# Harounnn/Clustering-Driven-Replication-Strategy

Hardware: AMD Instinct MI355X
Metric: Lloyd point-iters/sec (whole node) + achieved HBM GB/s, 100M files d=16 k=64 (higher is better)
Workload: dtype f64

## Files before the change

### clustering-driven-replication-strategy_amd/csrc/screen32b.hip

```cpp
#include "screen32_common.h"
#include "screen32_fix.h"

namespace cdr {

template <int Q, int MT>
__global__ __launch_bounds__(256, 4) void screen32b(S32BArgs B) {
  const S32PArgs& a = B.p;
  constexpr int QH = FixDims<Q>::QH;
  if (a.gate && a.gate[0] == 0) return;
  constexpr bool H1 = QH == 1;
  constexpr int kTile = H1 ? 512 : 1024;
  constexpr int kHalf = kTile / 2;
  constexpr int kPB = H1 ? 8 : 16;
  constexpr int NWH = kPB / 4;
  constexpr int kRow = 2 * kPB;
  typedef unsigned u4v __attribute__((ext_vector_type(4)));
  __shared__ __attribute__((aligned(16))) float c32s[64 * kPrStr + 128];
  float* const eb = c32s + 64 * kPrStr;
  float* const hc = eb + 64;
  constexpr size_t kQBytes = 4 * 2 * 2 * kTile + 4 * 128 * sizeof(int2);
  __shared__ __attribute__((aligned(16))) unsigned char qlds[kQBytes > kFixLdsBytes ? kQBytes : kFixLdsBytes];
  typedef unsigned char QRow[2][2 * kTile];
  QRow* qd = reinterpret_cast<QRow*>(qlds);
  int2 (*qm)[128] = reinterpret_cast<int2 (*)[128]>(qlds + 4 * 2 * 2 * kTile);
// ... 133 lines not shown
    const int label = (int)(bA & 63u);
    const float vb = __uint_as_float(bA & ~63u);
    const float vs = __uint_as_float(sA_ & ~63u);
    float thr = fmaf(vb, thr_rel, thr0);
    unsigned ua = __float_as_uint(hA), ub = __float_as_uint(hB);
    swap32(ua, ub);
    const float hsum = __uint_as_float(ua) + __uint_as_float(ub);
    const float hh = fmaf(hsum, 1.0f + 0x1p-18f, 0x1p-20f);
    const float hl = hsum * (1.0f - 0x1p-18f);
    const float dn = fmaf(0x1p-11f * (1.0f + 0x1p-9f), __builtin_amdgcn_sqrtf(hh), 0x1p-23f);
    {
      const float K = thr0 + hh - Dlo;
      const float Gs = fmaxf(vs + K, 0x1p-100f), Gb = fmaxf(fmaf(vb, thr_rel, K), 0x1p-100f);
      thr += 2.0f * (1.0f + 0x1p-19f) * dn * (__builtin_amdgcn_sqrtf(Gs) + __builtin_amdgcn_sqrtf(Gb));
    }
    const bool valid = lane < nvalid;
    const bool cert = vs > thr;
    const int pt = meta.x, ob = meta.y;
    const bool moved = valid && cert && label != ob;
    if (moved) {
      a.labels[pt] = label;
      a.lab8[pt] = (uint8_t)label;
    }
    const float gb = fmaf(vb, thr_rel, thr0 + hh - Dlo);
    const float gs = vs - ((thr0 + Dhi) - hl);
    const float u0 = fmaf(__builtin_amdgcn_sqrtf(fmaxf(gb, 0.0f)), 1.0f + 0x1p-19f, dn);
    const float l0 = fmaf(__builtin_amdgcn_sqrtf(fmaxf(gs, 0.0f)), 1.0f - 0x1p-19f, -dn);
    const float wl = __shfl(wdn_l, label);
    if (valid) B.zb[pt] = cert ? zb_pack(l0, u0, wl, (unsigned)label) : (kZbStale | (unsigned)ob);
    const bool unc = valid && !cert;
    const unsigned long long mv = __ballot(moved);
    const unsigned long long need = __ballot(unc);
    const int rm = __builtin_amdgcn_mbcnt_hi((unsigned)(mv >> 32),
                                             __builtin_amdgcn_mbcnt_lo((unsigned)mv, 0u));
    const int rn = __builtin_amdgcn_mbcnt_hi((unsigned)(need >> 32),
                                             __builtin_amdgcn_mbcnt_lo((unsigned)need, 0u));
    if (moved) mv_region[mv_used + rm] = int2{pt, ob | (label << 16)};
    if (unc) fb_region[fb_used + rn] = int2{pt, ob};
    mv_used += __popcll(mv);
    fb_used += __popcll(need);
  };
  int qh = 0, qn = 0;
  int qtot = 0, ttot = 0;
  auto process = [&](const Row& b, bool valid, int pt, int ao) __attribute__((always_inline)) {
    const float qa = dist2(b, ao);
    const float uba = fmaf(__builtin_amdgcn_sqrtf(qa), 1.0f + 0x1p-18f, eb[ao]);
    const float l0 = fmaf(hc[ao], 1.0f - 0x1p-22f, -uba);
    const bool keep = l0 > uba * (1.0f + 0x1p-20f);
    if (valid && keep) B.zb[pt] = zb_pack(l0, uba, __shfl(wdn_l, ao), (unsigned)ao);
#ifdef CDR_EXPERIMENTS
    const bool q = valid && !keep && !(B.dbg & 8);
#else
    const bool q = valid && !keep;
#endif
    const unsigned long long m = __ballot(q);
    if (m) {
      if (q) {
        const int r = __builtin_amdgcn_mbcnt_hi((unsigned)(m >> 32),
                                                __builtin_amdgcn_mbcnt_lo((unsigned)m, 0u));
        const int slot = (qh + r) & 127;
        const int e = slot & 63;
        unsigned char* dst = qd[wv][slot >> 6] + (e >> 5) * kTile + (e & 31) * kPB;
        if constexpr (H1) {
          *reinterpret_cast<uint2*>(dst) = uint2{b.w[0], b.w[1]};
          *reinterpret_cast<uint2*>(dst + kHalf) = uint2{b.w[2], b.w[3]};
        } else {
          *reinterpret_cast<uint4*>(dst) = uint4{b.w[0], b.w[1], b.w[2], b.w[3]};
          *reinterpret_cast<uint4*>(dst + kHalf) = uint4{b.w[4], b.w[5], b.w[6], b.w[7]};
        }
        qm[wv][slot] = int2{pt, ao};
      }
      const int c = __popcll(m);
      qh = (qh + c) & 127;
      qn += c;
      qtot += c;
      if (qn >= 64) {
        drain(((qh - qn) & 127) >> 6, 64);
        qn -= 64;
      }
    }
  };
  unsigned* const fl = flist[wv];
  struct GB {
    Row r;
    int pt, ao;
    bool valid;
  };
  auto gload = [&](GB& g, int b, int cnt) __attribute__((always_inline)) {
    const int e = 64 * b + lane;
    g.valid = e < cnt;
    const unsigned ent = fl[g.valid ? e : 64 * b];
    const int64_t ci = wave + (int64_t)(ent >> 14) * nwaves;
    const int64_t pt = ci * kBChunk + ((ent >> 6) & 255);
    g.pt = (int)pt;
    g.ao = (int)(ent & 63);
    const u4v* src = reinterpret_cast<const u4v*>(B.XH + pt * kRow);
    const u4v q0 = __builtin_nontemporal_load(src);
    g.r.w[0] = q0.x; g.r.w[1] = q0.y; g.r.w[2] = q0.z; g.r.w[3] = q0.w;
    if constexpr (!H1) {
      const u4v q1 = __builtin_nontemporal_load(src + 1);
      g.r.w[4] = q1.x; g.r.w[5] = q1.y; g.r.w[6] = q1.z; g.r.w[7] = q1.w;
    }
  };
  auto phase2 = [&](int& cnt, bool last) __attribute__((always_inline)) {
    const int nb = last ? (cnt + 63) >> 6 : cnt >> 6;
    if (nb == 0) return;
    ttot += last ? cnt : nb * 64;
#ifdef CDR_EXPERIMENTS
    if (B.dbg & 4) {
      cnt = 0;
      return;
    }
#endif
    GB g[3];
    gload(g[0], 0, cnt);
    gload(g[1], nb > 1 ? 1 : 0, cnt);
    for (int b = 0; b < nb; b += 3) {
#pragma unroll
      for (int i = 0; i < 3; ++i) {
        const int nx = b + i + 2;
        gload(g[(i + 2) % 3], nx < nb ? nx : nb - 1, cnt);
        if (b + i < nb) process(g[i].r, g[i].valid, g[i].pt, g[i].ao);
      }
    }
    const int done = nb * 64;
    const int rem = last ? 0 : cnt - done;
    if (rem > 0) {
      const unsigned v = lane < rem ? fl[done + lane] : 0u;
      __builtin_amdgcn_wave_barrier();
      if (lane < rem) fl[lane] = v;
    }
    cnt = rem;
  };

  int cnt = 0;
  int64_t it = 0;
  for (int64_t C0 = wave; C0 < nchunks; C0 += (int64_t)kBPD * nwaves) {
#pragma unroll
    for (int i = 0; i < kBPD; ++i, ++it) {
      const int64_t Ci = C0 + (int64_t)i * nwaves;
      if (Ci >= nchunks) break;
      zload(zc[(i + kBPD - 1) % kBPD], Ci + (int64_t)(kBPD - 1) * nwaves);
      const u4v z = zc[i];
#pragma unroll
      for (int u = 0; u < 4; ++u) {
        const unsigned w = z[u];
        const unsigned lab = w & 63u;
#ifdef CDR_EXPERIMENTS
        const bool fail = (!(__uint_as_float(w & ~63u) > __shfl(wup_l, (int)lab)) || (B.dbg & 1)) &&
                          !(B.dbg & 16);
#else
        const bool fail = !(__uint_as_float(w & ~63u) > __shfl(wup_l, (int)lab)) || (B.dbg & 1);
#endif
        const unsigned long long m = __ballot(fail);
        if (m) {
          if (fail) {
            const int r = __builtin_amdgcn_mbcnt_hi((unsigned)(m >> 32),
                                                    __builtin_amdgcn_mbcnt_lo((unsigned)m, 0u));
            fl[cnt + r] = (unsigned)it << 14 | (unsigned)(4 * lane + u) << 6 | lab;
          }
          cnt += __popcll(m);
        }
      }
      if (cnt > kBList - kBChunk) phase2(cnt, false);
    }
  }
  phase2(cnt, true);
  if (qn > 0) drain(((qh - qn) & 127) >> 6, qn);
  if (lane == 0) {
    a.fb_count[wave] = fb_used;
    a.mv_count[wave] = mv_used;
    if (a.q_acc) a.q_acc[wave] += qtot;
    if (B.t_acc) B.t_acc[wave] += ttot;
  }
#ifdef CDR_EXPERIMENTS
  if (B.dbg & 2) return;
#endif
  if (!a.fuse) return;
  __syncthreads();
  const FixLds L(qlds);
  if (lane == 0) {
    L.s_mv[wv + 1] = mv_used;
    L.s_fb[wv + 1] = fb_used;
  }
  fixup_regions<Q, MT>(a.fx, blockIdx.x * 4, 4, blockIdx.x % kRunSlices, L, FixPlan{sA, sC});
}

template <int KPD>
__global__ __launch_bounds__(256) void screen32bz(S32BArgs B) {
  const S32PArgs& a = B.p;
  if (a.gate && a.gate[0] == 0) return;
  typedef unsigned u4v __attribute__((ext_vector_type(4)));
  constexpr int kZList = KPD * kBChunk + 64;
  __shared__ unsigned flist[4][kZList];
  const int t = threadIdx.x;
  const int lane = t & 63;
  const int wv = t >> 6;
  const int wave = __builtin_amdgcn_readfirstlane(blockIdx.x * 4 + wv);
  const int64_t nchunks = B.nchunks;
  int64_t wbase, wend;
  int wstride;
  bs_range(B, wv, wbase, wstride, wend);
  auto zload = [&](u4v& z, int64_t ci) __attribute__((always_inline)) {
    const int64_t cc = ci < nchunks ? ci : nchunks - 1;
    z = __builtin_nontemporal_load(reinterpret_cast<const u4v*>(B.zb + cc * kBChunk) + lane);
  };
  u4v zc[KPD];
#pragma unroll
  for (int i = 0; i < KPD - 1; ++i) zload(zc[i], wbase + (int64_t)i * wstride);
  const float wup_l = B.wup[lane];
  unsigned* const fl = flist[wv];
  uint32_t* const out = B.zl + (size_t)wave * B.zcap;
  int cnt = 0, total = 0;
  int it = 0;
  for (int64_t C0 = wbase; C0 < wend; C0 += (int64_t)KPD * wstride) {
#pragma unroll
    for (int i = 0; i < KPD; ++i, ++it) {
      const int64_t Ci = C0 + (int64_t)i * wstride;
      if (Ci >= wend) break;
      zload(zc[(i + KPD - 1) % KPD], Ci + (int64_t)(KPD - 1) * wstride);
      const u4v z = zc[i];
#pragma unroll
      for (int u = 0; u < 4; ++u) {
        const unsigned w = z[u];
        const unsigned lab = w & 63u;
        const bool fail = !(__uint_as_float(w & ~63u) > __shfl(wup_l, (int)lab)) || (B.dbg & 1);
        const unsigned long long m = __ballot(fail);
        if (m) {
          if (fail) {
            const int r = __builtin_amdgcn_mbcnt_hi((unsigned)(m >> 32),
                                                    __builtin_amdgcn_mbcnt_lo((unsigned)m, 0u));
            fl[cnt + r] = (unsigned)it << 14 | (unsigned)(4 * lane + u) << 6 | lab;
          }
          cnt += __popcll(m);
        }
      }
    }
    if (cnt >= 64) {
      const int full = cnt & ~63;
      __builtin_amdgcn_wave_barrier();
      for (int o = 0; o < full; o += 64) out[total + o + lane] = fl[o + lane];
      const int rem = cnt - full;
      const unsigned v = lane < rem ? fl[full + lane] : 0u;
      __builtin_amdgcn_wave_barrier();
      if (lane < rem) fl[lane] = v;
      total += full;
      cnt = rem;
    }
  }
  __builtin_amdgcn_wave_barrier();
  if (lane < cnt) out[total + lane] = fl[lane];
  if (lane == 0) B.zn[wave] = total + cnt;
}

__global__ void zb_reset_kernel(const uint8_t* __restrict__ lab8, uint32_t* __restrict__ zb,
                                int64_t n, int64_t n_pad, const long long* __restrict__ gate) {
  if (gate && gate[0] == 0) return;
  for (int64_t i = (int64_t)blockIdx.x * blockDim.x + threadIdx.x; i < n_pad;
       i += (int64_t)gridDim.x * blockDim.x)
    zb[i] = i < n ? (kZbStale | lab8[i]) : 0x7F000000u;
}

__global__ void zh_reset_kernel(const uint8_t* __restrict__ lab8, uint16_t* __restrict__ zh,
                                int64_t n, int64_t n_pad, const long long* __restrict__ gate) {
  if (gate && gate[0] == 0) return;
  for (int64_t i = (int64_t)blockIdx.x * blockDim.x + threadIdx.x; i < n_pad;
       i += (int64_t)gridDim.x * blockDim.x)
    zh[i] = i < n ? (uint16_t)lab8[i] : (uint16_t)kZ16Pad;
}

__device__ __forceinline__ unsigned zb16_rebase(unsigned w, float dg, int e0o, int e0n) {
  const unsigned c = w >> 6;
  if (c == 0u || c == 1023u) return w;
  const float t = zb16_dec((int)c, e0o) - dg;
  int cn = t > 0.0f ? zb16_code(t * (1.0f - 0x1p-22f), e0n) : -1;
  cn = cn < 0 ? 0 : (cn > 1022 ? 1022 : cn);
  return (unsigned)cn << 6 | (w & 63u);
}

__global__ __launch_bounds__(256) void zh_rebase_kernel(uint16_t* __restrict__ zh, int64_t n_pad,
                                                        const unsigned char* __restrict__ bt,
                                                        const long long* __restrict__ gate) {
  if (gate && gate[0] == 0) return;
  const int* hd = reinterpret_cast<const int*>(bt + kBndHdr);
  if (hd[3] == 0) return;
  __shared__ float dgs[64];
  if (threadIdx.x < 64) dgs[threadIdx.x] = reinterpret_cast<const float*>(bt + kBndDG)[threadIdx.x];
  __syncthreads();
  const int e0o = hd[1], e0n = hd[2];
  typedef unsigned u4v __attribute__((ext_vector_type(4)));
  u4v* z4 = reinterpret_cast<u4v*>(zh);
  for (int64_t i = (int64_t)blockIdx.x * blockDim.x + threadIdx.x; i < n_pad / 8;
       i += (int64_t)gridDim.x * blockDim.x) {
    u4v z = __builtin_nontemporal_load(z4 + i);
#pragma unroll
    for (int q = 0; q < 4; ++q) {
      const unsigned lo = z[q] & 0xFFFFu, hi = z[q] >> 16;
      z[q] = zb16_rebase(lo, dgs[lo & 63u], e0o, e0n) | zb16_rebase(hi, dgs[hi & 63u], e0o, e0n) << 16;
    }
    __builtin_nontemporal_store(z, z4 + i);
  }
}

__global__ __launch_bounds__(256) void zh_watch_kernel(uint16_t* __restrict__ zh, int64_t n_pad,
                                                       unsigned char* __restrict__ bt,
                                                       const long long* __restrict__ gate,
                                                       uint32_t* __restrict__ wl,
                                                       int32_t* __restrict__ wn, int wcap,
                                                       int wrange) {
  if (gate && gate[0] == 0) return;
  const int* hd = reinterpret_cast<const int*>(bt + kBndHdr);
  int* wh = reinterpret_cast<int*>(bt + kBndWatch);
  const bool reb = hd[3] != 0;
  if (!reb && (wh[kWFin] == kWatchList || wh[kWHold])) return;
  __shared__ float dgs[64];
  __shared__ unsigned hs[64];
  const int t = threadIdx.x, lane = t & 63;
  if (t < 64) {
    dgs[t] = reinterpret_cast<const float*>(bt + kBndDG)[t];
    hs[t] = reinterpret_cast<const unsigned*>(bt + kBndH)[t];
  }
  __syncthreads();
  if (blockIdx.x == 0) {
    if (t < 64) reinterpret_cast<unsigned*>(bt + kBndHL)[t] = hs[t];
    if (t == 0) {
      wh[kWMode] = kWatchList;
      wh[kWValid] = 1;
      wh[kWEpochs] += 1;
      if (reb) wh[kWCarried] += 1;
    }
  }
  const int e0o = hd[1], e0n = hd[2];
  typedef unsigned u4v __attribute__((ext_vector_type(4)));
  const int wave = blockIdx.x * 4 + (t >> 6);
  const int64_t p0 = (int64_t)wave * wrange;
  const int64_t p1 = p0 + wrange < n_pad ? p0 + wrange : n_pad;
  uint32_t* const out = wl + (size_t)wave * wcap;
  int cnt = 0;
  constexpr int kU = 4;
  for (int64_t c0 = p0; c0 < p1; c0 += kU * kZ16Chunk) {
    u4v z[kU];
#pragma unroll
    for (int i = 0; i < kU; ++i) {
      const int64_t ci = c0 + i * kZ16Chunk < p1 ? c0 + i * kZ16Chunk : c0;
      z[i] = __builtin_nontemporal_load(reinterpret_cast<const u4v*>(zh + ci) + lane);
    }
#pragma unroll
    for (int i = 0; i < kU; ++i) {
      const int64_t ci = c0 + i * kZ16Chunk;
      if (ci >= p1) break;
      if (reb) {
#pragma unroll
        for (int q = 0; q < 4; ++q) {
          const unsigned lo = z[i][q] & 0xFFFFu, hi = z[i][q] >> 16;
          z[i][q] = zb16_rebase(lo, dgs[lo & 63u], e0o, e0n) |
                    zb16_rebase(hi, dgs[hi & 63u], e0o, e0n) << 16;
        }
        __builtin_nontemporal_store(z[i], reinterpret_cast<u4v*>(zh + ci) + lane);
      }
      const unsigned off = (unsigned)(ci - p0) + 8u * (unsigned)lane;
#pragma unroll
      for (int u = 0; u < 8; ++u) {
        const unsigned w = (z[i][u >> 1] >> (16 * (u & 1))) & 0xFFFFu;
        const bool listed = (w >> 6) <= hs[w & 63u];
        const unsigned long long m = __ballot(listed);
        if (m) {
          const int r = cnt + __builtin_amdgcn_mbcnt_hi((unsigned)(m >> 32),
                                                        __builtin_amdgcn_mbcnt_lo((unsigned)m, 0u));
          if (listed && r < wcap) out[r] = (off + (unsigned)u) << 16 | w;
          cnt += __popcll(m);
        }
      }
    }
  }
  if (lane == 0) {
    wn[wave] = cnt < wcap ? cnt : wcap;
    if (cnt > wcap) wh[kWOvf] = 1;
  }
}

void zh_rebase(Ctx& c, const long long* gate) {
  if (!c.zb_valid || c.zb_fmt != 16 || !c.bnd_ok) return;
  if (c.watch_on)
    hipLaunchKernelGGL(zh_watch_kernel, dim3(c.watch_waves / 4), dim3(256), 0, c.stream,
                       c.zb.as<uint16_t>(), c.n_pad, static_cast<unsigned char*>(c.bnd.p), gate,
                       c.wl.as<uint32_t>(), c.wn.as<int32_t>(), c.watch_cap, c.watch_range);
  else
    hipLaunchKernelGGL(zh_rebase_kernel, dim3(2048), dim3(256), 0, c.stream, c.zb.as<uint16_t>(),
                       c.n_pad, reinterpret_cast<const unsigned char*>(c.bnd.p), gate);
  HIP_CHECK(hipGetLastError());
}

void bound_words_reset(bool z16, hipStream_t s, const uint8_t* lab8, void* zb, int64_t n,
                       int64_t n_pad, const long long* gate) {
  if (z16)
    hipLaunchKernelGGL(zh_reset_kernel, dim3(2048), dim3(256), 0, s, lab8,
                       static_cast<uint16_t*>(zb), n, n_pad, gate);
  else
    hipLaunchKernelGGL(zb_reset_kernel, dim3(2048), dim3(256), 0, s, lab8,
                       static_cast<uint32_t*>(zb), n, n_pad, gate);
}

int screen32b_blocks_per_cu(int Q, int MT) {
  static int cache[4][2] = {};
  int& nb = cache[Q - 1][MT - 1];
  if (!nb)
    dispatch_q_mt<4>(Q, MT, [&](auto q, auto m) {
      nb = occupancy_blocks(screen32b<decltype(q)::value, decltype(m)::value>, 0);
    });
  return nb;
}

void screen32b_launch(int Q, int MT, dim3 grid, hipStream_t s, const S32BArgs& p) {
  dispatch_q_mt<4>(Q, MT, [&](auto q, auto m) {
    hipLaunchKernelGGL((screen32b<decltype(q)::value, decltype(m)::value>), grid, dim3(256), 0, s, p);
  });
}

void screen32bz_launch(dim3 grid, hipStream_t s, const S32BArgs& p) {
  static const int pd = exp_env("CDR_S32BZ_PD") ? std::atoi(exp_env("CDR_S32BZ_PD")) : 8;
  if (pd == 4) hipLaunchKernelGGL(screen32bz<4>, grid, dim3(256), 0, s, p);
  else if (pd == 12) hipLaunchKernelGGL(screen32bz<12>, grid, dim3(256), 0, s, p);
  else hipLaunchKernelGGL(screen32bz<8>, grid, dim3(256), 0, s, p);
}

}
```

### clustering-driven-replication-strategy_amd/csrc/screen32bs_body.h

```cpp
  static_assert(!(SPLIT && WATCH) && (!WATCH || CDR_S32BS_LAZY), "the WATCH form: 2-byte words, lazy phase 2");
  const S32PArgs& a = B.p;
  const FixArgs& F = a.fx;
#ifdef CDR_EXPERIMENTS
  unsigned long long tp[8] = {__builtin_amdgcn_s_memrealtime(), 0, 0, 0, 0, 0, 0, 0};
#define CDR_TP(i) tp[i] = __builtin_amdgcn_s_memrealtime()
#else
#define CDR_TP(i)
#endif
  constexpr int QH = FixDims<Q>::QH;
  constexpr int DM = FixDims<Q>::DM;
#ifndef CDR_S32BS_DEFER
#define CDR_S32BS_DEFER 1
#endif
  constexpr bool DEFER = !SPLIT && CDR_S32BS_DEFER;
  if constexpr (!MERGED) {
  if (!SPLIT && B.dyn && blockIdx.x == 0 && threadIdx.x < 32)
    B.dyn[((B.dyn_par ^ 1) * 32 + threadIdx.x) * 32] = 0u;
  if (a.gate && a.gate[0] == 0) return;
  if constexpr (!SPLIT) {
    if (B.watch) {
      const bool list = B.watch[kWMode] == kWatchList && B.watch[kWOvf] == 0;
      if (list != WATCH) return;
      if (blockIdx.x == 0 && threadIdx.x == 0) {
        B.watch[WATCH ? kWListN : kWFullN] += 1;
        B.watch[kWLast] = WATCH ? kWatchList : kWatchFull;
      }
    }
  }
  }
  typedef unsigned u4v __attribute__((ext_vector_type(4)));
  typedef float f2 __attribute__((ext_vector_type(2)));
  float* const eb = c32s + 64 * kPrStr;
  float* const hc = eb + 64;
  const int t = threadIdx.x;
  const int lane = t & 63;
  const int wv = t >> 6;
  const int h = lane >> 5, p = lane & 31;
  const int wave = __builtin_amdgcn_readfirstlane(blockIdx.x * 4 + wv);
  const int64_t nchunks = B.nchunks;
  const int k = a.k, d = a.d, d1 = d + 1;
  if constexpr (MERGED) __builtin_assume(d > 4 * (Q - 1));
  uint32_t* const wlw = WATCH ? B.wl + (size_t)wave * B.wcap : nullptr;
  const int pbase = WATCH ? wave * B.wrange : 0;

  constexpr int CH = SPLIT ? kBChunk : kZ16Chunk;
  constexpr int SH = SPLIT ? 14 : 15;
  auto zload = [&](u4v& z, int64_t ci) __attribute__((always_inline)) {
    const int64_t cc = ci < nchunks ? ci : nchunks - 1;
    z = __builtin_nontemporal_load(reinterpret_cast<const u4v*>(B.zh + cc * kZ16Chunk) + lane);
  };
  int64_t wbase, wend;
  int wstride;
  int64_t rR0 = 0;
  int rsl = 0;
  bs_range(B, wv, wbase, wstride, wend, &rR0, &rsl);
  const bool dyn = !SPLIT && !WATCH && B.dyn != nullptr && B.slot_wg > 0;
  int swend = (int)wend, P0 = (int)wend, P1 = (int)wend;
  if (dyn) {
    const int spw = (int)((wend - rR0) * B.dyn_pct / 100 / wstride);
    swend = (int)rR0 + spw * wstride;
    const int xcd = blockIdx.x & 7;
    P0 = swend + (int)((wend - swend) * xcd / 8);
    P1 = swend + (int)((wend - swend) * (xcd + 1) / 8);
  }
  const int ebase = dyn ? (int)rR0 : (int)wbase;
  const int estride = dyn ? 1 : wstride;
  u4v zc[kBPD];

  constexpr int kPr4 = (64 * kPrStr + 128) / 4;
  static_assert(kPr4 <= 512 && MT * 2 * 64 <= 256, "prologue: two float4 per thread");
  const f4* prune4 = reinterpret_cast<const f4*>(a.prune);
  const f4 pv0 = prune4[t];
  const f4 pv1 = t + 256 < kPr4 ? prune4[t + 256] : f4{0.f, 0.f, 0.f, 0.f};
  h8 av = {};
  if (t < MT * 2 * 64) av = a.frag[t];
  float cv = 0.0f;
  const int cm = t >> 5, ci4 = (t >> 3) & 3, chh = (t >> 2) & 1, cc = t & 3;
  if (t < MT * 32) cv = a.cinit[(cm * 16 + ci4 * 4 + cc) * 64 + chh * 32];
  float wup_l = 0.0f, wnew_l;
  int e0n = 0;
  if constexpr (SPLIT) {
    wup_l = B.wup[lane];
    wnew_l = B.wdn[lane];
  } else {
    wnew_l = reinterpret_cast<const float*>(B.bt + kBndWdg)[lane];
    e0n = reinterpret_cast<const int*>(B.bt + kBndHdr)[2];
  }
  auto zput = [&](int pt, int sl, bool ok, float l0, float u0, float w, unsigned lab) __attribute__((always_inline)) {
    if constexpr (SPLIT) {
      B.zb[pt] = ok ? zb_pack(l0, u0, w, lab) : (kZbStale | lab);
    } else {
      const unsigned short w16 = ok ? zb16_pack(l0, u0, w, e0n, lab) : (unsigned short)lab;
      B.zh[pt] = w16;
      if constexpr (WATCH) wlw[sl] = (unsigned)(pt - pbase) << 16 | w16;
    }
  };
  const float msv = lane < d ? F.ms[lane] : 0.0f;
  const float thr0 = a.thr_dev ? a.thr_dev[0] : a.thr0, thr_rel = a.thr_rel;
  const float Dv = a.thr_dev ? a.thr_dev[1] : a.Dv;
  const float Dlo = Dv * (1.0f - 0x1p-19f), Dhi = Dv * (1.0f + 0x1p-19f);
  const float sig = F.sig;
  int wtotal = 0;
  unsigned tlv = 0;
  if constexpr (WATCH) {
    wtotal = B.wn[wave];
    if (t < 64) tlv = (B.dbg & 1) ? 1022u : reinterpret_cast<const unsigned*>(B.bt + kBndT)[t];
    const int lastl = (B.wcap >> 8) - 1;
    const u4v* const wl4 = reinterpret_cast<const u4v*>(wlw);
#pragma unroll
    for (int i = 0; i < kBPD; ++i) {
      __builtin_amdgcn_sched_barrier(0);
      zc[i] = wl4[(size_t)(i < lastl ? i : lastl) * 64 + lane];
    }
    __builtin_amdgcn_sched_barrier(0);
    if (t < 64) tls[t] = tlv;
  }
  reinterpret_cast<f4*>(c32s)[t] = pv0;
  if (t + 256 < kPr4) reinterpret_cast<f4*>(c32s)[t + 256] = pv1;
  if (t < MT * 2 * 64) sA[t] = av;
  if (t < MT * 32) sC[t] = cv;
  for (int e = t; e < 64 * 17; e += 256) mtab[e] = 0ull;
  if (t < 16) msl[t] = msv;
  if constexpr (!SPLIT && !WATCH) {
    if (t < 64) tls[t] = (B.dbg & 1) ? 1022u : reinterpret_cast<const unsigned*>(B.bt + kBndT)[t];
  }
  if constexpr (WATCH) wtotal = __builtin_amdgcn_readfirstlane(wtotal);
  __syncthreads();
  CDR_TP(1);

  int fb_used = 0, fb_cert = 0, mv_used = 0, qtot = 0, ttot = 0;
  const f4* XA4 = reinterpret_cast<const f4*>(F.XA);

  auto screen_m = [&](int m, const u4v (&v)[QH]) __attribute__((always_inline)) -> f16v {
    asm volatile("" ::: "memory");
    const h8 A0 = sA[(m * 2 + 0) * 64 + lane];
    const h8 A1 = sA[(m * 2 + 1) * 64 + lane];
    f16v acc;
#pragma unroll
    for (int i4 = 0; i4 < 4; ++i4) {
      const f4 c4v = *reinterpret_cast<const f4*>(sC + ((m * 4 + i4) * 2 + h) * 4);
#pragma unroll
      for (int i = 0; i < 4; ++i) acc[4 * i4 + i] = c4v[i];
    }
    const h8 BH = __builtin_bit_cast(h8, v[0]);
    acc = __builtin_amdgcn_mfma_f32_32x32x16_f16(A0, BH, acc, 0, 0, 0);
    if constexpr (QH == 2) {
      const h8 BL = __builtin_bit_cast(h8, v[QH - 1]);
      acc = __builtin_amdgcn_mfma_f32_32x32x16_f16(A0, BL, acc, 0, 0, 0);
    }
    return __builtin_amdgcn_mfma_f32_32x32x16_f16(A1, BH, acc, 0, 0, 0);
  };
  auto tile = [&](const u4v (&v)[QH], unsigned& bk, unsigned& sk) __attribute__((always_inline)) {
    unsigned b = 0xFFFFFFFFu, s = 0xFFFFFFFFu;
#pragma nounroll
    for (int m = 0; m < MT; ++m) {
      const f16v acc = screen_m(m, v);
      const unsigned rb = 32u * (unsigned)m;
      auto key = [&](int i) {
        return (__float_as_uint(acc[i]) & ~63u) | (rb + (unsigned)(8 * (i >> 2) + (i & 3)));
      };
#pragma unroll
      for (int q = 0; q < 16; q += 2) {
        const unsigned x = key(q), y = key(q + 1);
        unsigned tq;
        asm("v_med3_u32 %0, %1, %2, %3" : "=v"(tq) : "v"(b), "v"(x), "v"(y));
        asm("v_min3_u32 %0, %1, %2, %3" : "=v"(b) : "v"(b), "v"(x), "v"(y));
        s = min(s, tq);
      }
    }
    bk = b | ((unsigned)h << 2);
    sk = s | ((unsigned)h << 2);
  };
  auto cmask = [&](const u4v (&v)[QH], float tau) __attribute__((always_inline)) -> unsigned {
    unsigned r = 0;
#pragma nounroll
    for (int m = 0; m < MT; ++m) {
      const f16v acc = screen_m(m, v);
#pragma unroll
      for (int i = 0; i < 16; ++i) {
        const float kv = __uint_as_float(__float_as_uint(acc[i]) & ~63u);
        if (!(kv > tau)) r |= 1u << (16 * m + i);
      }
    }
    return r;
  };
  auto q32 = [&](const float (&xh)[DM], int j) __attribute__((always_inline)) -> float {
    const f4* c4 = reinterpret_cast<const f4*>(c32s + j * kPrStr);
    f2 acc = {0.0f, 0.0f};
#pragma unroll
    for (int q = 0; q < Q; ++q) {
      const f4 cq = c4[q];
#pragma unroll
      for (int u = 0; u < 2; ++u) {
        const f2 df = {xh[4 * q + 2 * u] - cq[2 * u], xh[4 * q + 2 * u + 1] - cq[2 * u + 1]};
        acc = __builtin_elementwise_fma(df, df, acc);
      }
    }
    return acc.x + acc.y;
  };
  struct GB {
    f4 x[Q];
    int pt, ao;
    int sl;
    bool valid;
  };
  auto split_tiles = [&](const float (&xh)[DM], u4v (&T0)[QH], u4v (&T1)[QH]) __attribute__((always_inline)) {
    unsigned hw[4 * QH], lw[4 * QH];
#pragma unroll
    for (int qq = 0; qq < 2 * QH; ++qq) {
      f4 xt = {0.f, 0.f, 0.f, 0.f};
      if (qq < Q) xt = f4{xh[4 * qq], xh[4 * qq + 1], xh[4 * qq + 2], xh[4 * qq + 3]};
      split4(xt, hw[2 * qq], hw[2 * qq + 1], lw[2 * qq], lw[2 * qq + 1]);
    }
    unsigned ad[4 * QH], bd[4 * QH];
    if constexpr (QH == 1) {
      ad[0] = hw[0]; ad[1] = hw[1]; ad[2] = lw[0]; ad[3] = lw[1];
      bd[0] = hw[2]; bd[1] = hw[3]; bd[2] = lw[2]; bd[3] = lw[3];
    } else {
#pragma unroll
      for (int i = 0; i < 4; ++i) {
        ad[i] = hw[i];
        ad[4 + i] = lw[i];
        bd[i] = hw[4 + i];
        bd[4 + i] = lw[4 + i];
      }
    }
#pragma unroll
    for (int i = 0; i < 4 * QH; ++i) swap32(ad[i], bd[i]);
#pragma unroll
    for (int u = 0; u < QH; ++u) {
      T0[u] = u4v{ad[4 * u], ad[4 * u + 1], ad[4 * u + 2], ad[4 * u + 3]};
      T1[u] = u4v{bd[4 * u], bd[4 * u + 1], bd[4 * u + 2], bd[4 * u + 3]};
    }
  };
  auto keys = [&](const u4v (&T0)[QH], const u4v (&T1)[QH], unsigned& b, unsigned& s) __attribute__((always_inline)) {
    unsigned bB, sB;
    tile(T0, b, s);
    tile(T1, bB, sB);
    swap32(b, bB);
    swap32(s, sB);
    merge_top2(b, s, bB, sB);
  };
  auto rowhat = [&](const f4 (&x)[Q], float (&xh)[DM]) __attribute__((always_inline)) {
#pragma unroll
    for (int f = 0; f < DM; ++f) xh[f] = f < d ? fmaf(x[f >> 2][f & 3], sig, msl[f]) : 0.0f;
  };
  auto move = [&](bool live, int pt, int ao, int lab, const f4* row) __attribute__((always_inline)) {
    const bool moved = live && lab != ao;
    const unsigned long long mm = __ballot(moved);
    if (!mm) return;
    if (moved) {
      a.labels[pt] = lab;
      a.lab8[pt] = (uint8_t)lab;
      f4 xr[Q];
#pragma unroll
      for (int q = 0; q < Q; ++q) xr[q] = row ? row[q] : XA4[(int64_t)pt * Q + q];
#pragma unroll
      for (int f = 0; f < DM; ++f) {
        if (f < d) {
          const long long v = __double2ll_rn((double)xr[f >> 2][f & 3] * F.fx);
          atomicAdd(&mtab[lab * d1 + f], (unsigned long long)v);
          atomicAdd(&mtab[ao * d1 + f], (unsigned long long)-v);
        }
      }
      atomicAdd(&mtab[lab * d1 + d], 1ull);
      atomicAdd(&mtab[ao * d1 + d], ~0ull);
    }
    mv_used += __popcll(mm);
  };
  int2* fb_region = a.fb_list + (size_t)wave * a.cap;
  auto rec_x = [&](int pt, int sl) __attribute__((always_inline)) -> int {
    return WATCH ? (int)((unsigned)(pt - pbase) << 16 | (unsigned)sl) : pt;
  };
  auto near_tie = [&](bool live, int ao, unsigned bkey, const float (&xh)[DM],
                      const u4v (&T0)[QH], const u4v (&T1)[QH], const f4 (&xr)[Q], float xx,
                      bool& c2, float& u0, float& l0) __attribute__((always_inline)) -> int {
    const double* cs = F.cent;
    const float tau = fmaf(__uint_as_float(bkey & ~63u), thr_rel, thr0);
    unsigned mine[2], other[2];
#pragma unroll
    for (int tt = 0; tt < 2; ++tt) {
      const float tau_t = __shfl(tau, 32 * tt + p);
      const unsigned r = cmask(tt == 0 ? T0 : T1, tau_t);
      mine[tt] = r;
      other[tt] = (unsigned)__shfl_xor((int)r, 32);
    }
    int lab = ao;
    c2 = false;
    u0 = l0 = 0.0f;
    if (live) {
      unsigned long long cand = 0;
      const unsigned mh0 = h == 0 ? mine[0] : other[1], mh1 = h == 0 ? other[0] : mine[1];
#pragma unroll
      for (int hh = 0; hh < 2; ++hh) {
        unsigned mmk = hh ? mh1 : mh0;
        while (mmk) {
          const int bb = __builtin_ctz(mmk);
          mmk &= mmk - 1;
          const int m = bb >> 4, i = bb & 15;
          cand |= 1ull << (32 * m + 8 * (i >> 2) + 4 * hh + (i & 3));
        }
      }
      if (k < 64) cand &= (1ull << k) - 1;
      const float xu = fmaf(xx, 1.0f + 0x1p-19f, 0x1p-120f);
      const float xl = xx * (1.0f - 0x1p-19f);
      const float dn32 = fmaf(0x1p-24f * (1.0f + 0x1p-20f), __builtin_amdgcn_sqrtf(xu), 0x1p-120f);
      float ub = INFINITY, lo_other = INFINITY, lb_best = INFINITY, rbest = INFINITY;
      int jb = 0;
      bool bad = false;
      unsigned long long cm2 = cand;
      while (cm2) {
        const int j = __builtin_ctzll(cm2);
        cm2 &= cm2 - 1;
        float nc;
        {
          const float zr[DM] = {};
          nc = q32(zr, j);
        }
        const float ec = fmaf(0x1p-24f * (1.0f + 0x1p-18f),
                              __builtin_amdgcn_sqrtf(nc * (1.0f + 0x1p-19f)), 0x1p-120f);
        const float e2 = (dn32 + ec) * (1.0f + 0x1p-20f);
        const float r = __builtin_amdgcn_sqrtf(q32(xh, j));
        const float U = fmaf(r, 1.0f + 0x1p-19f, e2), L = fmaf(r, 1.0f - 0x1p-19f, -e2);
        bad = bad || !(U == U) || !(L == L);
        if (r < rbest) {
          lo_other = fminf(lo_other, lb_best);
          rbest = r;
          ub = U;
          lb_best = L;
          jb = j;
        } else {
          lo_other = fminf(lo_other, L);
        }
      }
      const float gs = tau - ((thr0 + Dhi) - xl);
      const float lnc = fmaf(__builtin_amdgcn_sqrtf(fmaxf(gs, 0.0f)), 1.0f - 0x1p-19f, -dn32);
      c2 = !bad && rbest < INFINITY && lo_other > ub * (1.0f + 0x1p-20f);
      if (c2) {
        lab = jb;
        u0 = ub;
        l0 = fminf(lo_other, lnc);
      } else {
        float x[16];
#pragma unroll
        for (int f = 0; f < 16; ++f) x[f] = f < DM ? xr[f >> 2][f & 3] : 0.0f;
        double sb = INFINITY, rb = INFINITY;
        int jmin = 0x7fffffff;
        while (cand) {
          const int j = __builtin_ctzll(cand);
          cand &= cand - 1;
          const double sq = np_sqdist16(x, cs + j * d, d);
          if (sq < sb) {
            const double rt = sqrt(sq);
            sb = sq;
            if (rt < rb) {
              rb = rt;
              jmin = j;
            }
          }
        }
        lab = jmin >= k ? 0 : jmin;
      }
    }
    return lab;
  };
  auto norm2 = [&](const float (&xh)[DM]) __attribute__((always_inline)) -> float {
    f2 acc = {0.0f, 0.0f};
#pragma unroll
    for (int f = 0; f < DM; f += 2) {
      const f2 v = {xh[f], xh[f + 1]};
      acc = __builtin_elementwise_fma(v, v, acc);
    }
    return acc.x + acc.y;
  };
  auto kcase = [&](float xx, float vb, float vs, float& u0, float& l0) __attribute__((always_inline)) {
    const float xu = fmaf(xx, 1.0f + 0x1p-19f, 0x1p-120f);
    const float xl = xx * (1.0f - 0x1p-19f);
    const float dn32 = fmaf(0x1p-24f * (1.0f + 0x1p-20f), __builtin_amdgcn_sqrtf(xu), 0x1p-120f);
    const float gb = fmaf(vb, thr_rel, thr0 + xu - Dlo);
    const float gs = vs - ((thr0 + Dhi) - xl);
    u0 = fmaf(__builtin_amdgcn_sqrtf(fmaxf(gb, 0.0f)), 1.0f + 0x1p-19f, dn32);
    l0 = fmaf(__builtin_amdgcn_sqrtf(fmaxf(gs, 0.0f)), 1.0f - 0x1p-19f, -dn32);
  };
  auto decide = [&](const GB& g) __attribute__((always_inline)) {
    const bool valid = g.valid;
    const int pt = g.pt, ao = g.ao, sl = g.sl;
    float xh[DM];
    rowhat(g.x, xh);
    const float qa = q32(xh, ao);
    const float xx = norm2(xh);
    bool need;
    if (B.direct) {
      const f4 nv = reinterpret_cast<const f4*>(c32s + ao * kPrStr)[4];
      const int n1 = __float_as_int(nv[kPrN1 - 16]), n2 = __float_as_int(nv[kPrN2 - 16]);
      const float xu = fmaf(xx, 1.0f + 0x1p-19f, 0x1p-120f);
      const float dn32 = fmaf(0x1p-24f * (1.0f + 0x1p-20f), __builtin_amdgcn_sqrtf(xu), 0x1p-120f);
      int jb = ao;
      float rbest = 0.0f, ub = 0.0f, lb_best = 0.0f, lo = INFINITY, ua = 0.0f;
      bool bad = false;
#pragma unroll
      for (int c = 0; c < 3; ++c) {
        const int jn = c == 0 ? ao : (c == 1 ? n1 : n2);
        const bool none = (unsigned)jn >= 64u;
        const int j = none ? ao : jn;
        const float q = c == 0 ? qa : (none ? INFINITY : q32(xh, j));
        const float ec = c == 0 ? nv[kPrEc - 16] : c32s[j * kPrStr + kPrEc];
        const float e2 = (dn32 + ec) * (1.0f + 0x1p-20f);
        const float r = __builtin_amdgcn_sqrtf(q);
        const float U = fmaf(r, 1.0f + 0x1p-19f, e2), L = fmaf(r, 1.0f - 0x1p-19f, -e2);
        bad = bad || !(U == U) || !(L == L);
        if (c == 0) {
          rbest = r;
          ub = ua = U;
          lb_best = L;
        } else if (r < rbest) {
          lo = fminf(lo, lb_best);
          rbest = r;
          ub = U;
          lb_best = L;
          jb = j;
        } else {
          lo = fminf(lo, L);
        }
      }
      const float l0 = fminf(lo, fmaf(nv[kPrH3 - 16], 1.0f - 0x1p-22f, -ua));
      const bool dec = !bad && l0 > ub * (1.0f + 0x1p-20f);
      const float w_b = __shfl(wnew_l, jb);
      if (valid && dec) zput(pt, sl, true, l0, ub, w_b, (unsigned)jb);
      move(valid && dec, pt, ao, jb, g.x);
      need = valid && !dec;
    } else {
      const float uba = fmaf(__builtin_amdgcn_sqrtf(qa), 1.0f + 0x1p-18f, eb[ao]);
      const float l0P = fmaf(hc[ao], 1.0f - 0x1p-22f, -uba);
      const bool keep = l0P > uba * (1.0f + 0x1p-20f);
      const float w_ao = __shfl(wnew_l, ao);
      if (valid && keep) zput(pt, sl, true, l0P, uba, w_ao, (unsigned)ao);
      need = valid && !keep;
    }
    const unsigned long long nm = __ballot(need);
    if (!nm) return;
    qtot += __popcll(nm);
#ifdef CDR_EXPERIMENTS
    if (B.dbg & 8) return;
#endif
    if constexpr (DEFER) {
      if (B.direct && __popcll(nm) < kDirectDense) {
        if (need) {
          const int r = __builtin_amdgcn_mbcnt_hi((unsigned)(nm >> 32),
                                                  __builtin_amdgcn_mbcnt_lo((unsigned)nm, 0u));
          fb_region[fb_used + r] = int2{rec_x(pt, sl), (int)(kNotScreened | (unsigned)ao)};
        }
        fb_used = __builtin_amdgcn_readfirstlane(fb_used + __popcll(nm));
        return;
      }
    }
    unsigned bA, sA_;
    u4v T0[QH], T1[QH];
    split_tiles(xh, T0, T1);
    keys(T0, T1, bA, sA_);
    const int label = (int)(bA & 63u);
    const float vb = __uint_as_float(bA & ~63u);
    const float vs = __uint_as_float(sA_ & ~63u);
    const bool cert = vs > fmaf(vb, thr_rel, thr0);
    const bool unc = need && !cert;
    const float w_lab = __shfl(wnew_l, label);
    if (need && cert) {
      float u0, l0;
      kcase(xx, vb, vs, u0, l0);
      zput(pt, sl, true, l0, u0, w_lab, (unsigned)label);
    }
    const unsigned long long um = __ballot(unc);
    if constexpr (DEFER) {
    if (um) {
      if (unc) {
        const int r = __builtin_amdgcn_mbcnt_hi((unsigned)(um >> 32),
                                                __builtin_amdgcn_mbcnt_lo((unsigned)um, 0u));
        fb_region[fb_used + r] = int2{rec_x(pt, sl), (int)((bA & ~63u) | (unsigned)ao)};
      }
      fb_used += __popcll(um);
    }
    move(need && cert, pt, ao, label, nullptr);
    } else {
    int labf = label;
    if (um) {
#ifdef CDR_EXPERIMENTS
      if (!(B.dbg & 2)) {
#endif
      bool c2;
      float u0, l0;
      const int lab = near_tie(unc, ao, bA, xh, T0, T1, g.x, xx, c2, u0, l0);
      const float wl = __shfl(wnew_l, lab);
      if (unc) {
        labf = lab;
        zput(pt, sl, c2, l0, u0, wl, (unsigned)lab);
      }
#ifdef CDR_EXPERIMENTS
      } else if (unc) {
        labf = ao;
      }
#endif
      fb_used += __popcll(um);
    }
    move(need, pt, ao, labf, g.x);
    }
  };

  unsigned* const fl = flist[wv];
  constexpr int kWL = kSList / 2;
  constexpr int LS = WATCH ? kWL : kSList;
  constexpr int kRoom = WATCH ? 256 : CH;
  auto gfill = [&](GB& g, int e) __attribute__((always_inline)) {
    const unsigned ent = fl[e];
    int64_t pt;
    if constexpr (WATCH) {
      pt = pbase + (int)(ent >> 16);
      g.sl = (int)fl[kWL + e];
    } else {
      const int64_t ci = ebase + (int64_t)(ent >> SH) * estride;
      pt = ci * CH + ((ent >> 6) & (CH - 1));
      g.sl = 0;
    }
    g.pt = (int)pt;
    g.ao = (int)(ent & 63);
#pragma unroll
    for (int q = 0; q < Q; ++q) g.x[q] = __builtin_nontemporal_load(XA4 + pt * Q + q);
  };
  auto gload = [&](GB& g, int b, int cnt) __attribute__((always_inline)) {
    const int e = 64 * b + lane;
    g.valid = e < cnt;
    gfill(g, g.valid ? e : 64 * b);
  };
  auto phase2 = [&](int& cnt, bool last) __attribute__((always_inline)) {
    const int nb = last ? (cnt + 63) >> 6 : cnt >> 6;
    if (nb == 0) return;
    ttot += last ? cnt : nb * 64;
#ifdef CDR_EXPERIMENTS
    if (B.dbg & 4) {
      cnt = 0;
      return;
    }
#endif
#if CDR_S32BS_DEPTH >= 3
    GB cur, nxt, nx2;
    gload(cur, 0, cnt);
    gload(nxt, nb > 1 ? 1 : 0, cnt);
#pragma nounroll
    for (int b = 0; b < nb; ++b) {
      gload(nx2, b + 2 < nb ? b + 2 : nb - 1, cnt);
      decide(cur);
      cur = nxt;
      nxt = nx2;
    }
#else
    GB cur, nxt;
    gload(cur, 0, cnt);
#pragma nounroll
    for (int b = 0; b < nb; ++b) {
      gload(nxt, b + 1 < nb ? b + 1 : nb - 1, cnt);
      decide(cur);
      cur = nxt;
    }
#endif
    const int done = nb * 64;
    const int rem = last ? 0 : cnt - done;
    if (rem > 0) {
      const unsigned v = lane < rem ? fl[done + lane] : 0u;
      __builtin_amdgcn_wave_barrier();
      if (lane < rem) fl[lane] = v;
    }
// ... 350 lines not shown
```

Before: 2755 billion.

## Double-buffer watch-kernel loads and stage list writes through LDS for coalesced output

```diff
diff --git a/clustering-driven-replication-strategy_amd/csrc/screen32b.hip b/clustering-driven-replication-strategy_amd/csrc/screen32b.hip
--- a/clustering-driven-replication-strategy_amd/csrc/screen32b.hip
+++ b/clustering-driven-replication-strategy_amd/csrc/screen32b.hip
@@ -459,6 +459,86 @@
   }
 }
 
+constexpr int kWStage = 1024;
+template <bool REB>
+__device__ __forceinline__ int zh_watch_range(uint16_t* __restrict__ zh, int64_t p0, int64_t p1,
+                                              const float* dgs, const unsigned* hs, int e0o,
+                                              int e0n, uint32_t* __restrict__ out, int wcap,
+                                              unsigned* stg, int lane) {
+  typedef unsigned u4v __attribute__((ext_vector_type(4)));
+  constexpr int kU = 4;
+  const int nch = (int)((p1 - p0 + kZ16Chunk - 1) / kZ16Chunk);
+  if (nch <= 0) return 0;
+  u4v* const zw = reinterpret_cast<u4v*>(zh + p0) + lane;
+  int cnt = 0;
+  int done = 0;
+  auto group = [&](u4v (&zc)[kU], u4v (&zx)[kU], int c0) __attribute__((always_inline)) {
+#pragma unroll
+    for (int i = 0; i < kU; ++i) {
+      const int c = c0 + kU + i;
+      zx[i] = __builtin_nontemporal_load(zw + (size_t)(c < nch ? c : nch - 1) * 64);
+      __builtin_amdgcn_sched_barrier(0);
+    }
+#pragma unroll
+    for (int i = 0; i < kU; ++i) {
+      const int c = c0 + i;
+      if (c >= nch) break;
+      u4v w = zc[i];
+      if constexpr (REB) {
+#pragma unroll
+        for (int q = 0; q < 4; ++q) {
+          const unsigned lo = w[q] & 0xFFFFu, hi = w[q] >> 16;
+          w[q] = zb16_rebase(lo, dgs[lo & 63u], e0o, e0n) |
+                 zb16_rebase(hi, dgs[hi & 63u], e0o, e0n) << 16;
+        }
+        __builtin_nontemporal_store(w, zw + (size_t)c * 64);
+      }
+      unsigned m = 0;
+#pragma unroll
+      for (int u = 0; u < 8; ++u) {
+        const unsigned x = (w[u >> 1] >> (16 * (u & 1))) & 0xFFFFu;
+        m |= (unsigned)((x >> 6) <= hs[x & 63u]) << u;
+      }
+      if (__ballot(m != 0u)) {
+        const unsigned off = (unsigned)c * kZ16Chunk + 8u * (unsigned)lane;
+        int tot = 0;
+#pragma unroll
+        for (int u = 0; u < 8; ++u) {
+          const bool listed = (m >> u) & 1u;
+          const unsigned long long bm = __ballot(listed);
+          const unsigned r = (unsigned)(cnt + tot) +
+                             __builtin_amdgcn_mbcnt_hi((unsigned)(bm >> 32),
+                                                       __builtin_amdgcn_mbcnt_lo((unsigned)bm, 0u));
+          const unsigned x = (w[u >> 1] >> (16 * (u & 1))) & 0xFFFFu;
+          if (listed) stg[r & (kWStage - 1)] = (off + (unsigned)u) << 16 | x;
+          tot += __popcll(bm);
+        }
+        cnt = __builtin_amdgcn_readfirstlane(cnt + tot);
+        __builtin_amdgcn_wave_barrier();
+        for (; done + 64 <= cnt; done += 64) {
+          const unsigned v = stg[(done & (kWStage - 1)) + lane];
+          if (done + lane < wcap) out[done + lane] = v;
+        }
+        __builtin_amdgcn_wave_barrier();
+      }
+    }
+  };
+  u4v za[kU], zb[kU];
+#pragma unroll
+  for (int i = 0; i < kU; ++i)
+    za[i] = __builtin_nontemporal_load(zw + (size_t)(i < nch ? i : nch - 1) * 64);
+  for (int c0 = 0;;) {
+    group(za, zb, c0);
+    c0 += kU;
+    if (c0 >= nch) break;
+    group(zb, za, c0);
+    c0 += kU;
+    if (c0 >= nch) break;
+  }
+  if (done + lane < cnt && done + lane < wcap) out[done + lane] = stg[(done & (kWStage - 1)) + lane];
+  return cnt;
+}
+
 __global__ __launch_bounds__(256) void zh_watch_kernel(uint16_t* __restrict__ zh, int64_t n_pad,
                                                        unsigned char* __restrict__ bt,
                                                        const long long* __restrict__ gate,
@@ -472,6 +552,7 @@
   if (!reb && (wh[kWFin] == kWatchList || wh[kWHold])) return;
   __shared__ float dgs[64];
   __shared__ unsigned hs[64];
+  __shared__ unsigned stg[4][kWStage];
   const int t = threadIdx.x, lane = t & 63;
   if (t < 64) {
     dgs[t] = reinterpret_cast<const float*>(bt + kBndDG)[t];
@@ -488,48 +569,13 @@
     }
   }
   const int e0o = hd[1], e0n = hd[2];
-  typedef unsigned u4v __attribute__((ext_vector_type(4)));
   const int wave = blockIdx.x * 4 + (t >> 6);
   const int64_t p0 = (int64_t)wave * wrange;
   const int64_t p1 = p0 + wrange < n_pad ? p0 + wrange : n_pad;
   uint32_t* const out = wl + (size_t)wave * wcap;
-  int cnt = 0;
-  constexpr int kU = 4;
-  for (int64_t c0 = p0; c0 < p1; c0 += kU * kZ16Chunk) {
-    u4v z[kU];
-#pragma unroll
-    for (int i = 0; i < kU; ++i) {
-      const int64_t ci = c0 + i * kZ16Chunk < p1 ? c0 + i * kZ16Chunk : c0;
-      z[i] = __builtin_nontemporal_load(reinterpret_cast<const u4v*>(zh + ci) + lane);
-    }
-#pragma unroll
-    for (int i = 0; i < kU; ++i) {
-      const int64_t ci = c0 + i * kZ16Chunk;
-      if (ci >= p1) break;
-      if (reb) {
-#pragma unroll
-        for (int q = 0; q < 4; ++q) {
-          const unsigned lo = z[i][q] & 0xFFFFu, hi = z[i][q] >> 16;
-          z[i][q] = zb16_rebase(lo, dgs[lo & 63u], e0o, e0n) |
-                    zb16_rebase(hi, dgs[hi & 63u], e0o, e0n) << 16;
-        }
-        __builtin_nontemporal_store(z[i], reinterpret_cast<u4v*>(zh + ci) + lane);
-      }
-      const unsigned off = (unsigned)(ci - p0) + 8u * (unsigned)lane;
-#pragma unroll
-      for (int u = 0; u < 8; ++u) {
-        const unsigned w = (z[i][u >> 1] >> (16 * (u & 1))) & 0xFFFFu;
-        const bool listed = (w >> 6) <= hs[w & 63u];
-        const unsigned long long m = __ballot(listed);
-        if (m) {
-          const int r = cnt + __builtin_amdgcn_mbcnt_hi((unsigned)(m >> 32),
-                                                        __builtin_amdgcn_mbcnt_lo((unsigned)m, 0u));
-          if (listed && r < wcap) out[r] = (off + (unsigned)u) << 16 | w;
-          cnt += __popcll(m);
-        }
-      }
-    }
-  }
+  unsigned* const sw = stg[t >> 6];
+  const int cnt = reb ? zh_watch_range<true>(zh, p0, p1, dgs, hs, e0o, e0n, out, wcap, sw, lane)
+                      : zh_watch_range<false>(zh, p0, p1, dgs, hs, e0o, e0n, out, wcap, sw, lane);
   if (lane == 0) {
     wn[wave] = cnt < wcap ? cnt : wcap;
     if (cnt > wcap) wh[kWOvf] = 1;
diff --git a/clustering-driven-replication-strategy_amd/csrc/screen32bs_body.h b/clustering-driven-replication-strategy_amd/csrc/screen32bs_body.h
--- a/clustering-driven-replication-strategy_amd/csrc/screen32bs_body.h
+++ b/clustering-driven-replication-strategy_amd/csrc/screen32bs_body.h
@@ -252,9 +252,24 @@
     if (moved) {
       a.labels[pt] = lab;
       a.lab8[pt] = (uint8_t)lab;
+#ifdef CDR_EXPERIMENTS
+      const int reps = (B.dbg & 32) ? 3 : 1;
+#pragma nounroll
+      for (int rep = 0; rep < reps; ++rep) {
+        if (rep) {
+          const int sw = lab;
+          lab = ao;
+          ao = sw;
+        }
+#endif
       f4 xr[Q];
 #pragma unroll
       for (int q = 0; q < Q; ++q) xr[q] = row ? row[q] : XA4[(int64_t)pt * Q + q];
+#ifdef CDR_EXPERIMENTS
+#pragma unroll
+      for (int q = 0; q < Q; ++q)
+        asm volatile("" : "+v"(xr[q][0]), "+v"(xr[q][1]), "+v"(xr[q][2]), "+v"(xr[q][3]));
+#endif
 #pragma unroll
       for (int f = 0; f < DM; ++f) {
         if (f < d) {
@@ -265,6 +280,9 @@
       }
       atomicAdd(&mtab[lab * d1 + d], 1ull);
       atomicAdd(&mtab[ao * d1 + d], ~0ull);
+#ifdef CDR_EXPERIMENTS
+      }
+#endif
     }
     mv_used += __popcll(mm);
   };
```

Result: no change. 2751 billion (-0.1%).
